# BurntSushi/aho-corasick

Hardware: NVIDIA H100
Metric: haystack_scan_throughput (higher is better)
Workload: dtype u8

## Files before the change

aho-corasick_b200/csrc/acb_api.cu:

```cuda
#include <cuda_runtime.h>

#include <algorithm>
#include <chrono>
#include <cstdio>
#include <cstdlib>
#include <cstring>
#include <atomic>
#include <pthread.h>
#include <condition_variable>
#include <functional>
#include <mutex>
#include <thread>
#include <new>
#include <optional>
#include <vector>

#include "../../include/acb200.h"
#include "../../include/acb200_debug.h"
#include "acb_build.hpp"
#include "acb_comm.hpp"
#include "acb_device.cuh"
#include "acb_plan.hpp"

using acb::DfaDev;
// ... 53 lines not shown
  cudaStream_t stream = nullptr, copy_stream = nullptr;
  cudaEvent_t ev0 = nullptr, ev1 = nullptr, ev2 = nullptr, ev3 = nullptr;
  DevBuf<uint64_t> d_keys[2];
  DevBuf<uint32_t> d_pids[2];
  uint64_t tuple_cap() const { return d_keys[0].cap; }
  DevBuf<unsigned long long> d_counter;
  PinnedBuf<unsigned long long> h_counter;
  DevBuf<uint8_t> d_temp;
  DevBuf<uint8_t> d_hay;
  DevBuf<uint64_t> d_scratch;
  DevBuf<uint8_t> d_flags;
  DevBuf<uint64_t> d_rec;
  PinnedBuf<uint64_t> h_rec;
  acg_stats stats{};
  PinnedBuf<uint8_t> h_stage[2];
  cudaEvent_t stage_ev[2] = {nullptr, nullptr};
  DevBuf<uint64_t> d_doc_offs;
  DevBuf<unsigned long long> d_doc_counts, d_doc_incl;
  DevBuf<uint8_t> d_doc_flags;
  DevBuf<uint64_t> d_rep;
  DevBuf<uint8_t> d_out;
  DevBuf<uint8_t> d_sdocs;
  DevBuf<uint64_t> d_soffs;
  DevBuf<uint64_t> d_held;
};

}

struct acg_dfa {
  HostDfa h;
  std::vector<uint16_t> depth16;
  acb::PrefilterPlan pf;
  uint32_t* d_bitmap = nullptr;
  uint2* d_amap = nullptr;
  bool has_empty = false;
  uint32_t max_list_len = 0;
  bool on_device = false;
  bool dev_touched = false;
  int device = -1;
  uint32_t* d_trans = nullptr;
  uint8_t* d_classes = nullptr;
  uint32_t* d_moff = nullptr;
  uint32_t* d_mpids = nullptr;
  uint32_t* d_plens = nullptr;
  uint16_t* d_depth16 = nullptr;
  DfaDev dev{};
  int engine_override = ACG_ENGINE_AUTO;
  uint64_t pipeline_chunk = 64ull << 20;
  mutable bool bytescan_inert = false;
  uint32_t experiment = 0;
  mutable std::mutex mu;
  static constexpr size_t kMaxWorkspaces = 4;
  mutable std::vector<Workspace*> ws_all, ws_free;
  mutable std::condition_variable ws_cv;
  mutable acg_stats last_stats{};
};

struct acg_streams {
  const acg_dfa* a = nullptr;
  uint64_t n = 0, back = 0;
  bool overlapping = false;
  bool replace = false;
  uint64_t* d_state = nullptr;
  uint8_t* d_tail = nullptr;
  uint64_t* d_rep = nullptr;
};
// ... 173 lines not shown
  std::vector<uint32_t>().swap(fp.edge_off);
  std::vector<uint8_t>().swap(fp.edge_class);
  std::vector<uint32_t>().swap(fp.edge_to);
  return ACG_OK;
}

int upload(acg_dfa* a) {
  int ndev = 0;
  if (cudaGetDeviceCount(&ndev) != cudaSuccess || ndev == 0) {
    cudaGetLastError();
    return ACG_E_NO_DEVICE;
  }
  CK(cudaGetDevice(&a->device));
  a->dev_touched = true;
  HostDfa& h = a->h;
  auto up = [&](auto** dptr, const void* src, size_t bytes) -> cudaError_t {
    cudaError_t e = cudaMalloc(reinterpret_cast<void**>(dptr), std::max<size_t>(bytes, 16));
    if (e != cudaSuccess) return e;
    if (bytes) e = cudaMemcpy(*dptr, src, bytes, cudaMemcpyHostToDevice);
    return e;
  };
  if (h.fill.valid) {
    int rc = fill_table_on_device(a);
    if (rc) return rc;
  } else {
    CK(up(&a->d_trans, h.trans.data(), h.trans.size() * 4));
  }
  CK(up(&a->d_classes, h.classes, 256));
  CK(up(&a->d_moff, h.match_offsets.data(), h.match_offsets.size() * 4));
  CK(up(&a->d_mpids, h.match_pids.data(), h.match_pids.size() * 4));
  CK(up(&a->d_plens, h.pattern_lens.data(), h.pattern_lens.size() * 4));
  CK(up(&a->d_depth16, a->depth16.data(), a->depth16.size() * 2));
  if (a->pf.supported && !a->pf.bitmap.empty()) CK(up(&a->d_bitmap, a->pf.bitmap.data(), a->pf.bitmap.size() * 4));
  if (a->pf.supported && !a->pf.amap.empty()) CK(up(&a->d_amap, a->pf.amap.data(), a->pf.amap.size() * 8));
  DfaDev& d = a->dev;
  d.trans = a->d_trans;
  d.classes = a->d_classes;
  d.match_offsets = a->d_moff;
  d.match_pids = a->d_mpids;
  d.pattern_lens = a->d_plens;
  d.depth16 = a->d_depth16;
  d.stride2 = h.stride2;
  d.max_match_id = h.max_match_id;
  d.start_unanchored_id = h.start_unanchored_id;
  d.start_anchored_id = h.start_anchored_id;
  d.max_pattern_len = uint32_t(std::min<uint64_t>(h.max_pattern_len, UINT32_MAX));
  d.min_pattern_len = uint32_t(std::min<uint64_t>(h.min_pattern_len, UINT32_MAX));
  d.amap = a->d_amap;
  acb::plan_device_fields(a->pf, d);
  a->on_device = true;
  return ACG_OK;
}

int reserve_tuples(Workspace& w, uint64_t cap) {
  return reserve_all(cap, w.d_keys[0], w.d_pids[0], w.d_keys[1], w.d_pids[1]);
}

template <class F>
int cub_call(Workspace& w, F f) {
  size_t tb = 0;
  CK(f(nullptr, tb));
  int rc = w.d_temp.reserve(std::max<size_t>(tb, 16));
  if (rc) return rc;
  tb = w.d_temp.cap;
  CK(f(w.d_temp, tb));
  return ACG_OK;
// ... 50 lines not shown
  if (const char* e = getenv("ACB_EMU_BUCKETSHIFT")) { shift = std::min<uint32_t>(uint32_t(atoi(e)), max_shift); min_shift = 1; }
  if (const char* e = getenv("ACB_EMU_BUCKETLOG")) log = std::min<uint32_t>(uint32_t(std::max(atoi(e), 0)), acb::kOrderLog);
#endif
  if (shift < min_shift) return b;
  while ((n_bytes >> shift) + 1 > acb::kMaxBuckets) {
    if (shift >= max_shift) return b;
    ++shift;
  }
  b.shift = shift;
  b.n = uint32_t((n_bytes >> shift) + 1);
  b.log = log;
  b.tie_bits = tie_bits;
  return b;
}

int enqueue_prefilter_range(const acg_dfa* a, const uint8_t* d_hay, uint64_t readable,
                            uint64_t span_start, uint64_t span_end, uint64_t scan_lo,
                            uint64_t scan_hi, int mode, int dev_sms, const BucketPlan& bp,
                            const DocBatch* docs) {
  Workspace& w = cur_ws();
  const acb::PrefilterPlan& pf = a->pf;
  const uintptr_t base = reinterpret_cast<uintptr_t>(d_hay);
  uint64_t lo = scan_lo + ((16 - ((base + scan_lo) & 15)) & 15);
  const uint64_t limit = std::min<uint64_t>(scan_hi, readable >= 20 ? readable - 20 : 0);
  uint64_t hi = lo;
  if (limit > lo) hi = lo + ((limit - lo) & ~15ull);
  if (lo > scan_hi) { lo = scan_hi; hi = scan_hi; }
  acb::PrefilterLaunch p;
  p.hay = d_hay;
  p.hay_len = readable;
  p.span_start = span_start;
  p.span_end = span_end;
  p.bitmap = a->d_bitmap;
  p.log_bits = pf.log_bits;
  p.k = pf.k;
  p.stride = pf.stride;
  p.geom = pf.wide ? 1 : 0;
  p.dyn = (a->experiment & ACG_EXP_STATIC_TILES) ? 0 : ((a->experiment & ACG_EXP_GLOBAL_TILES) ? 2 : 1);
  p.kmask = pf.kmask;
  p.fold = pf.fold;
  p.mult = pf.mult;
  p.mult3 = pf.mult3;
  p.key_shift = pf.key_shift;
  p.shift = pf.shift;
  p.dense = pf.dense ? 1 : 0;
  p.brute = pf.brute ? 1 : 0;
  p.mode = mode == 1 ? 1 : 0;
  p.first_only = mode == 2 ? 1 : 0;
  p.dup_shift = pf.dup_shift;
  p.scan_lo = scan_lo;
  p.scan_hi = scan_hi;
  p.region_lo = lo;
  p.region_hi = hi;
  p.keys = w.d_keys[0];
  p.pids = w.d_pids[0];
  p.counter = w.d_counter;
  p.cap = w.tuple_cap();
  p.bucket_shift = bp.shift;
  p.bucket_log = bp.log;
  p.bucket_slots = bp.slots();
  p.doc_offsets = docs ? docs->d_offsets : nullptr;
  p.n_docs = docs ? docs->n : 0;
  p.bs_n = 0;
  for (int i = 0; i < 3; ++i) { p.bs_needle[i] = 0; p.bs_back[i] = 0; }
  if (pf.bs_n && !a->bytescan_inert && !(a->experiment & ACG_EXP_NO_BYTESCAN)) {
    p.bs_n = pf.bs_n;
// ... 1745 lines not shown
    std::memcpy(h.classes, d->byte_classes, 256);
    h.max_special_id = d->max_special_id;
    h.max_match_id = d->max_match_id;
    h.start_unanchored_id = d->start_unanchored_id;
    h.start_anchored_id = d->start_anchored_id;
    const size_t nms = size_t(d->max_match_id >> d->stride2) - 1;
    h.match_offsets.assign(d->match_offsets, d->match_offsets + nms + 1);
    h.match_pids.assign(d->match_pids, d->match_pids + h.match_offsets[nms]);
    h.pattern_lens.assign(d->pattern_lens, d->pattern_lens + d->n_patterns);
    h.match_kind = int(d->match_kind);
    h.start_kind = int(d->start_kind);
    h.prefilter_kind = int(d->prefilter_kind);
    h.reported_kind = ACG_KIND_DFA;
    h.min_pattern_len = d->min_pattern_len;
    h.max_pattern_len = d->max_pattern_len;
    h.state_len = d->trans_len >> d->stride2;
    derive_metadata(a);
  } catch (const std::bad_alloc&) {
    delete a;
    return ACG_E_NOMEM;
  }
  int rc = upload(a);
  if (rc != ACG_OK && rc != ACG_E_NO_DEVICE) { acg_dfa_free(a); return rc; }
  *out = a;
  return ACG_OK;
}

void acg_dfa_free(acg_dfa* a) {
  if (!a) return;
  if (a->on_device || a->dev_touched) {
    DeviceGuard guard(a->device);
    for (Workspace* w : a->ws_all) { destroy_workspace(*w); delete w; }
    cudaFree(a->d_trans); cudaFree(a->d_classes); cudaFree(a->d_moff); cudaFree(a->d_mpids);
    cudaFree(a->d_plens); cudaFree(a->d_depth16); cudaFree(a->d_bitmap); cudaFree(a->d_amap);
  }
  delete a;
}

namespace {
int fetch_table(const acg_dfa* a) {
  HostDfa& h = const_cast<acg_dfa*>(a)->h;
  if (!h.fill.valid || !h.trans.empty()) return ACG_OK;
  if (!a->d_trans) return ACG_E_NO_DEVICE;
  std::lock_guard<std::mutex> lock(a->mu);
  if (!h.trans.empty()) return ACG_OK;
  DeviceGuard guard(a->device);
  std::vector<uint32_t> t(size_t(h.trans_len));
  if (cudaMemcpy(t.data(), a->d_trans, t.size() * 4, cudaMemcpyDeviceToHost) != cudaSuccess) {
    cudaGetLastError();
    return ACG_E_CUDA;
  }
  h.trans.swap(t);
  return ACG_OK;
}

}

int acg_dfa_table(const acg_dfa* a, acg_dfa_desc* o) {
  if (!a || !o) return ACG_E_INVALID_ARG;
  if (int rc = fetch_table(a)) return rc;
  const HostDfa& h = a->h;
  o->trans = h.trans.data();
  o->trans_len = h.trans.size();
  o->stride2 = h.stride2;
  o->alphabet_len = h.alphabet_len;
  std::memcpy(o->byte_classes, h.classes, 256);
  o->max_special_id = h.max_special_id;
// ... 14 lines not shown

uint64_t acg_dfa_state_len(const acg_dfa* a) { return a ? a->h.state_len : 0; }
int acg_kind(const acg_dfa* a) { return a ? a->h.reported_kind : 0; }
int acg_match_kind(const acg_dfa* a) { return a ? a->h.match_kind : 0; }
int acg_start_kind(const acg_dfa* a) { return a ? a->h.start_kind : 0; }
uint64_t acg_patterns_len(const acg_dfa* a) { return a ? a->h.pattern_lens.size() : 0; }
uint64_t acg_min_pattern_len(const acg_dfa* a) { return a ? a->h.min_pattern_len : 0; }
uint64_t acg_max_pattern_len(const acg_dfa* a) { return a ? a->h.max_pattern_len : 0; }
uint64_t acg_memory_usage(const acg_dfa* a) {
  if (!a) return 0;
  const HostDfa& h = a->h;
  return h.trans_len * 4 + (h.match_offsets.size() - 1) * 24 + h.match_pids.size() * 4 +
         h.pattern_lens.size() * 4;
}
int acg_prefilter_kind(const acg_dfa* a) { return a ? a->h.prefilter_kind : 0; }
int acg_packed_variant(const acg_dfa* a, int* fat, int* mask_len) {
  if (!a || !a->h.packed.active) return 0;
  if (fat) *fat = a->h.packed.fat;
  if (mask_len) *mask_len = a->h.packed.mask_len;
  return 1;
}

int acg_debug_prefilter_plan(const acg_dfa* a, acg_prefilter_plan* out) {
  if (!a || !out) return ACG_E_INVALID_ARG;
  const acb::PrefilterPlan& pf = a->pf;
  *out = acg_prefilter_plan{};
  out->supported = pf.supported ? 1 : 0;
  out->brute = pf.brute ? 1 : 0;
  out->dense = pf.dense ? 1 : 0;
  out->stride = int32_t(pf.stride);
  out->wide = pf.wide ? 1 : 0;
  out->k = pf.k; out->kmask = pf.kmask; out->fold = pf.fold;
  out->mult = pf.mult; out->mult3 = pf.mult3; out->key_shift = pf.key_shift; out->shift = pf.shift; out->log_bits = pf.log_bits;
  out->bitmap = pf.bitmap.data(); out->bitmap_words = pf.bitmap.size();
  out->amap = pf.amap.data(); out->amap_log = pf.amap_log;
  out->depth16 = a->depth16.data(); out->n_rows = a->depth16.size();
  out->dup_shift = pf.dup_shift;
  out->bs_n = (pf.bs_n && !a->bytescan_inert) ? pf.bs_n : 0;
  for (int i = 0; i < 3; ++i) { out->bs_byte[i] = pf.bs_byte[i]; out->bs_back[i] = pf.bs_back[i]; }
  return ACG_OK;
}

int acg_debug_set_pipeline_chunk(acg_dfa* a, uint64_t bytes) {
  if (!a || bytes < 4096 || (bytes & 4095)) return ACG_E_INVALID_ARG;
  a->pipeline_chunk = bytes;
  return ACG_OK;
}

int acg_debug_set_experiment(acg_dfa* a, uint32_t flags) {
  if (!a || (flags & ~uint32_t(ACG_EXP_KEY24 | ACG_EXP_STATIC_TILES | ACG_EXP_NO_BYTESCAN | ACG_EXP_GLOBAL_TILES))) return ACG_E_INVALID_ARG;
  std::lock_guard<std::mutex> lock(a->mu);
  const uint32_t changed = a->experiment ^ flags;
  a->experiment = flags;
  if (changed & ACG_EXP_KEY24) {
    const size_t old_words = a->pf.bitmap.size();
    a->pf = acb::plan_prefilter(a->h, a->depth16, (flags & ACG_EXP_KEY24) != 0);
    if (a->on_device && a->d_bitmap && a->pf.supported) {
      if (a->pf.bitmap.size() != old_words) return ACG_E_INVALID_ARG;
      DeviceGuard guard(a->device);
      if (cudaMemcpy(a->d_bitmap, a->pf.bitmap.data(), old_words * 4, cudaMemcpyHostToDevice) != cudaSuccess) {
        cudaGetLastError();
        return ACG_E_CUDA;
      }
    }
  }
  return ACG_OK;
}

int acg_set_engine(acg_dfa* a, int engine) {
  if (!a || engine < ACG_ENGINE_AUTO || engine > ACG_ENGINE_SEQUENTIAL) return ACG_E_INVALID_ARG;
  a->engine_override = engine;
  return ACG_OK;
}
static acg_stats stats_for(const acg_dfa* a) {
  if (tls_stats_owner == a) return tls_stats;
  std::lock_guard<std::mutex> lk(a->mu);
  return a->last_stats;
}
int acg_last_engine(const acg_dfa* a) { return a ? stats_for(a).engine : 0; }
int acg_last_stats(const acg_dfa* a, acg_stats* out) {
  if (!a || !out) return ACG_E_INVALID_ARG;
  *out = stats_for(a);
  return ACG_OK;
}

int acg_find_overlapping(const acg_dfa* a, const uint8_t* hay, uint64_t hay_len, uint64_t span_start,
                         uint64_t span_end, int anchored, acg_match* out, uint64_t cap,
                         uint64_t* n_out) {
  return overlapping_impl(a, hay, false, hay_len, span_start, span_end, anchored, out, cap, n_out,
                          nullptr, nullptr);
}
int acg_find_overlapping_dev(const acg_dfa* a, const void* d_hay, uint64_t hay_len,
                             uint64_t span_start, uint64_t span_end, acg_match* out, uint64_t cap,
// ... 600 lines not shown
```

aho-corasick_b200/csrc/acb_device.cuh:

```cuda
#pragma once
#include <cuda_runtime.h>
#include <stdint.h>

namespace acb {

constexpr int kTieBits = 24;
constexpr uint64_t kTieMask = (1ull << kTieBits) - 1;
constexpr uint64_t kInvalidKey = ~0ull;

struct MatchSpan {
  uint64_t start, end;
};
__host__ __device__ __forceinline__ MatchSpan decode_key(uint64_t key, uint32_t pid, int key_mode, uint64_t span_start,
                                                         const uint32_t* pattern_lens) {
  const uint64_t at = span_start + (key >> kTieBits);
  if (key_mode == 1) return MatchSpan{at, at + (key & kTieMask)};
  return MatchSpan{at - pattern_lens[pid], at};
}

struct TupleList {
  const uint64_t* keys;
  const uint32_t* pids;
  const uint32_t* pattern_lens;
  uint64_t n;
// ... 192 lines not shown
cudaError_t launch_stream_flush(const StreamLaunch& p, const uint64_t* ids, uint64_t n_ids,
                                const uint64_t* out_offsets, uint8_t* out, cudaStream_t s);

struct LookLaunch {
  StreamLaunch st;
  const uint64_t* ids;
  uint64_t n_rows;
  const uint64_t* cand_offsets;
  const uint8_t* cand_classes;
  uint64_t n_cands;
  uint64_t* keys;
  uint32_t* rows;
  uint64_t* skeys;
  uint32_t* srows;
  unsigned long long* heads;
  uint64_t* row_u;
  uint8_t* out;
  int sm_count;
};
cudaError_t launch_look_state(const DfaDev& dfa, const LookLaunch& p, cudaStream_t s);
cudaError_t launch_look_heads(const LookLaunch& p, cudaStream_t s);
cudaError_t launch_look_compact(const LookLaunch& p, cudaStream_t s);
cudaError_t launch_look_mask(const DfaDev& dfa, const LookLaunch& p, cudaStream_t s);
cudaError_t launch_look_copy(const LookLaunch& p, cudaStream_t s);

cudaError_t launch_check_offsets(const uint64_t* offs, uint64_t n_docs, uint64_t hay_len,
                                 unsigned long long* result, cudaStream_t s);

struct PrefilterLaunch {
  const uint8_t* hay;
  uint64_t hay_len;
  uint64_t span_start, span_end;
  const uint32_t* bitmap;
  uint32_t log_bits;
  uint32_t k;
  uint32_t stride;
  uint16_t geom;
  uint32_t kmask;
  uint32_t fold;
  uint32_t mult;
  uint32_t mult3;
  uint32_t shift;
  int dense;
  int brute;
  int mode;
  int first_only;
  uint32_t dup_shift;
  uint64_t scan_lo, scan_hi;
  uint64_t region_lo, region_hi;
  uint64_t* keys;
  uint32_t* pids;
  unsigned long long* counter;
  uint64_t cap;
  uint32_t dyn;
  uint32_t bs_n;
  uint32_t bs_needle[3];
  uint32_t bs_back[3];
  uint32_t key_shift;
  uint32_t bucket_shift;
  uint32_t bucket_log;
  uint64_t bucket_slots;
  const uint64_t* doc_offsets;
  uint64_t n_docs;
};
cudaError_t launch_prefilter(const DfaDev& dfa, const PrefilterLaunch& p, int sm_count, cudaStream_t s);
cudaError_t launch_bytescan(const DfaDev& dfa, const PrefilterLaunch& p, int sm_count, cudaStream_t s);
// ... 50 lines not shown
```

aho-corasick_b200/csrc/acb_fingerprint.cuh:

```cuda
#pragma once
#include <stdint.h>

#ifdef __CUDACC__
#define ACB_FP_FN __host__ __device__ __forceinline__
#else
#define ACB_FP_FN inline
#endif

namespace acb {

constexpr uint32_t kNarrowLogBits = 20, kWideLogBits = 17;
ACB_FP_FN constexpr uint32_t bloom_shift(uint32_t log_bits) { return 35 - log_bits; }
constexpr uint64_t kDenseGrams = 8192;
constexpr uint32_t kMult = 0x9E3779B1u;

ACB_FP_FN uint32_t bloom_hash2(uint32_t x) {
  x ^= x >> 16;
  x *= 0x7feb352du;
  x ^= x >> 15;
  x *= 0x846ca68bu;
  x ^= x >> 16;
  return x;
}

ACB_FP_FN uint32_t bloom_hash3(uint32_t x) {
  x ^= x >> 15;
  x *= 0x2c1b3c6du;
  x ^= x >> 12;
  x *= 0x297a2d39u;
  x ^= x >> 15;
  return x;
}

ACB_FP_FN uint32_t bloom_bit(uint32_t h, uint32_t sel, uint32_t shift) { return (h >> shift) * 8 + (sel & 7); }
ACB_FP_FN uint32_t key_mult(uint32_t mult3, uint32_t key_shift) { return mult3 << key_shift; }

ACB_FP_FN uint32_t dense_word(uint32_t lo, uint32_t shift) { return lo >> (shift + 2); }
ACB_FP_FN uint32_t dense_bit_a(uint32_t hi) { return hi & 31; }
ACB_FP_FN uint32_t dense_bit_b(uint32_t hi) { return (hi >> 5) & 31; }

ACB_FP_FN int bit_width(uint64_t v) { int b = 0; for (; v; v >>= 1) ++b; return b; }

ACB_FP_FN uint32_t amap_log_for(uint64_t n_keys) { return uint32_t(bit_width((n_keys * 4 - 1) | 15)); }
ACB_FP_FN uint32_t amap_slot(uint32_t key, uint32_t amap_shift) { return bloom_hash3(key) >> amap_shift; }
ACB_FP_FN uint32_t amap_next(uint32_t slot, uint32_t amap_mask) { return (slot + 1) & amap_mask; }
// ... 4 lines not shown
```

aho-corasick_b200/csrc/acb_plan.hpp:

```cpp
#pragma once
#include <algorithm>

#include "acb_build.hpp"
#include "acb_device.cuh"
#include "acb_fingerprint.cuh"

namespace acb {

struct PrefilterPlan {
  bool supported = false;
  uint32_t k = 0, kmask = 0, fold = 0, mult = 1, mult3 = 1, shift = 0, log_bits = 0;
  uint32_t stride = 1;
  uint32_t key_shift = 8;
  bool wide = false;
  bool brute = false;
  uint32_t dup_shift = 0;
  std::vector<uint32_t> bitmap;
  bool dense = false;
  std::vector<uint64_t> amap;
  uint32_t amap_log = 0;
  uint32_t bs_n = 0;
  uint8_t bs_byte[3] = {0, 0, 0};
  uint8_t bs_back[3] = {0, 0, 0};
};

namespace plan_detail {

inline void set_bit(std::vector<uint32_t>& bm, uint32_t bit) { bm[bit >> 5] |= 1u << (bit & 31); }
inline uint32_t test_bit(const std::vector<uint32_t>& bm, uint32_t bit) { return (bm[bit >> 5] >> (bit & 31)) & 1u; }

inline std::vector<uint32_t> bloom_bitmap(const std::vector<uint32_t>& grams, uint32_t log_bits) {
  const uint32_t shift = bloom_shift(log_bits);
  std::vector<uint32_t> bm(size_t(1) << (log_bits - 5), 0u);
  for (uint32_t g : grams) {
    const uint32_t h1 = g * kMult, h2 = bloom_hash2(g);
    set_bit(bm, bloom_bit(h1, h1, shift));
    set_bit(bm, bloom_bit(h2, h2, shift));
  }
  return bm;
}

struct DenseBits { uint32_t word, mask; };
inline DenseBits dense_bits(uint32_t g, uint32_t shift) {
  const uint64_t prod = uint64_t(g) * kMult;
  const uint32_t hi = uint32_t(prod >> 32);
  return {dense_word(uint32_t(prod), shift), (1u << dense_bit_a(hi)) | (1u << dense_bit_b(hi))};
}

struct Alphabets {
  std::vector<uint8_t> at[4];
// ... 110 lines not shown
    std::fill(pf.bitmap.begin(), pf.bitmap.end(), 0u);
    for (uint32_t g : best_set) { const DenseBits d = dense_bits(g, pf.shift); pf.bitmap[d.word] |= d.mask; }
    const Alphabets alpha = alphabets(best_set, pf.k);
    fill = double(count_passes([&](auto& next) {
             uint32_t g = 0;
             for (uint32_t j = 0; j < pf.k; ++j) g |= uint32_t(alpha.at[j][(next() >> 33) % alpha.at[j].size()]) << (8 * j);
             const DenseBits d = dense_bits(g, pf.shift);
             return uint32_t((pf.bitmap[d.word] & d.mask) == d.mask);
           })) / kTrials;
  }
  pf.brute = fill > 0.25;
  pf.supported = true;
  if (!pf.brute && pf.k == 4 && !dense) {
    std::vector<uint32_t> g3;
    g3.reserve(best_set.size() * 2);
    const uint32_t f3 = pf.fold & 0x00FFFFFFu;
    for (uint32_t g : best_set) {
      g3.push_back((g & 0x00FFFFFFu) | f3);
      g3.push_back((g >> 8) | f3);
    }
    std::sort(g3.begin(), g3.end());
    g3.erase(std::unique(g3.begin(), g3.end()), g3.end());
    const Alphabets alpha = alphabets(g3, 3);
    const double n_bits_set = double(g3.size()) + 2.0 * double(best_set.size());
    const double true3 = double(g3.size()) / alpha.space;
    const double pass1 = n_bits_set / double(uint64_t(1) << pf.log_bits) + true3;
    if (pass1 < 0.07) {
      pf.stride = 2;
      pf.wide = n_bits_set / double(uint64_t(1) << kWideLogBits) + true3 < 0.01;
      if (pf.wide) {
        pf.log_bits = kWideLogBits;
        pf.shift = bloom_shift(kWideLogBits);
        pf.bitmap = bloom_bitmap(best_set, kWideLogBits);
      }
      pf.key_shift = key24 ? 8 : 5;
      std::vector<uint32_t> keys1;
      if (key24) {
        keys1 = g3;
      } else {
        for (const Item& it : level[4]) {
          const uint32_t g = it.gram;
          keys1.push_back(((g & 0x00FFFFFFu) | f3) | (((g >> 24) & 7u) << 24));
          uint32_t xs = 0;
          if (it.row >= 2 && (it.row << s2) <= h.max_match_id) {
            const uint32_t lo = h.match_offsets[it.row - 2], hi = h.match_offsets[it.row - 1];
            if (lo < hi && h.pattern_lens[h.match_pids[lo]] == 4) xs = 0xFF;
          }
          if (xs != 0xFF)
            for_each_edge(it.row, [&](uint32_t b, uint32_t nr) {
              if (depth16[nr] == 5) xs |= 1u << (b & 7);
            });
          for (uint32_t x = 0; x < 8; ++x)
            if (xs >> x & 1) keys1.push_back(((g >> 8) | f3) | (x << 24));
        }
        std::sort(keys1.begin(), keys1.end());
        keys1.erase(std::unique(keys1.begin(), keys1.end()), keys1.end());
      }
      static const uint32_t kCand[] = {0x1B873593u, 0x27D4EB2Fu, 0x165667B1u, 0x9E3779B1u, 0x2C1B3C6Du,
                                       0xB5297A4Du, 0x85EBCA6Bu, 0x5BD1E995u, 0x7FEB352Du, 0xCC9E2D51u,
                                       0x1B56C4E9u, 0xC2B2AE35u};
      auto key_bit = [&](uint32_t g, uint32_t m) { return bloom_bit(g * key_mult(m, pf.key_shift), g, pf.shift); };
      uint32_t best_m = kCand[0];
      uint64_t best_pass = UINT64_MAX;
      std::vector<uint32_t> trial;
      for (uint32_t m : kCand) {
        trial = pf.bitmap;
        for (uint32_t g : keys1) set_bit(trial, key_bit(g, m));
        const uint64_t pass = count_passes([&](auto& next) {
          const uint64_t x = next();
          const uint32_t r = uint32_t(x >> 33);
          uint32_t g = uint32_t(alpha.at[0][r % alpha.at[0].size()]) |
                       uint32_t(alpha.at[1][(r >> 10) % alpha.at[1].size()]) << 8 |
                       uint32_t(alpha.at[2][(r >> 20) % alpha.at[2].size()]) << 16;
          if (!key24) g |= uint32_t((x >> 20) & 7) << 24;
          return test_bit(trial, key_bit(g, m));
        });
        if (pass < best_pass) { best_pass = pass; best_m = m; }
      }
      pf.mult3 = best_m;
      for (uint32_t g : keys1) set_bit(pf.bitmap, key_bit(g, best_m));
    }
  }
  pf.dense = !pf.brute && dense;
  const std::vector<Item>& paths = level[pf.k];
  if (!paths.empty() && paths.size() <= (4u << 20)) {
    pf.amap_log = amap_log_for(paths.size());
    pf.amap.assign(size_t(1) << pf.amap_log, 0ull);
    const uint32_t shift = 32 - pf.amap_log, mask = (1u << pf.amap_log) - 1;
    for (const Item& it : paths) {
      const uint32_t key = it.gram & pf.kmask;
      uint32_t slot = amap_slot(key, shift);
      while (pf.amap[slot] != 0 && uint32_t(pf.amap[slot]) != key) slot = amap_next(slot, mask);
      pf.amap[slot] = amap_entry(key, it.row << s2);
    }
  }
  if (h.prefilter_kind == kPreStartBytes || h.prefilter_kind == kPreRareBytes) {
    if (h.pre_n) {
      if (std::all_of(h.pre_back, h.pre_back + h.pre_n, [](uint8_t back) { return back == 0; })) {
        pf.bs_n = h.pre_n;
        std::copy(h.pre_byte, h.pre_byte + h.pre_n, pf.bs_byte);
      }
    } else if (h.prefilter_kind == kPreStartBytes && !level[1].empty() && grams[1].size() <= 3) {
      pf.bs_n = uint32_t(grams[1].size());
      std::copy(grams[1].begin(), grams[1].end(), pf.bs_byte);
    }
  }
  return pf;
}

inline void plan_device_fields(const PrefilterPlan& pf, DfaDev& d) {
  d.amap_shift = pf.amap_log ? 32 - pf.amap_log : 0;
  d.amap_mask = pf.amap_log ? (1u << pf.amap_log) - 1 : 0;
  d.amap_k = pf.k;
// ... 5 lines not shown
```

aho-corasick_b200/csrc/acb_prefilter.cu:

```cuda
#include "acb_device.cuh"
#include "acb_fingerprint.cuh"
#ifndef ACB_PTX_HEADER
#define ACB_PTX_HEADER "acb_ptx.cuh"
#endif
#include ACB_PTX_HEADER

#include <cstdio>
#include <cstdlib>
#include <type_traits>

#include <cub/device/device_scan.cuh>
#include <cub/device/device_select.cuh>

namespace acb {
namespace {

enum : int { kGeomNarrow = 0, kGeomWide = 1 };
template <int GEOM> struct PfGeom {
  static constexpr int kThreads = GEOM == kGeomNarrow ? 1024 : 512;
  static constexpr int kWarps = kThreads / 32;
  static constexpr int kGroups = GEOM == kGeomNarrow ? 2 : 4;
  static constexpr int kTile = kGroups * 512;
  static constexpr int kStageBytes = kTile + 16;
  static constexpr int kMinCtas = GEOM == kGeomWide ? 2 : 1;
  static constexpr uint32_t kLogBits = GEOM == kGeomWide ? kWideLogBits : kNarrowLogBits;
};
template <bool DENSE> struct PfCfg {
  static constexpr int kSlots = 256;
  static constexpr int kQ2 = DENSE ? 64 : 96;
};

#ifdef ACB_EMULATE
static const uint32_t kWinShift = getenv("ACB_EMU_WINSHIFT") ? (uint32_t)atoi(getenv("ACB_EMU_WINSHIFT")) : 31u;
#else
constexpr uint32_t kWinShift = 31;
#endif

constexpr int kPfStages = 2;

template <int GEOM, int STRIDE> struct PfPass {
  static constexpr bool kPair = STRIDE == 2 && GEOM == kGeomNarrow;
  static constexpr int kStages = kPair ? 1 : kPfStages;
  static constexpr int kGroups = PfGeom<GEOM>::kGroups * (kPair ? 2 : 1);
  static constexpr int kTile = kGroups * 512;
  static_assert(kStages * (kTile + 16) <= kPfStages * PfGeom<GEOM>::kStageBytes, "a step's tiles fit the warp's ring");
};

template <bool BUCKETED = true>
struct Emitter {
  uint64_t* g_keys;
  uint32_t* g_pids;
  unsigned long long* g_counter;
  uint64_t cap;
  uint32_t bucket_shift, bucket_log;
  uint64_t bucket_slots;
  __device__ __forceinline__ void emit(uint64_t key, uint32_t pid) {
    const unsigned m = __activemask();
    const int leader = __ffs(m) - 1;
    const int lane = threadIdx.x & 31;
    const bool bucketed = BUCKETED && bucket_shift != 0;
    unsigned long long* cnt = g_counter;
// ... 97 lines not shown
}

template <int MODE, class EM>
__device__ __forceinline__ void verify_at(const DfaDev& d, const PrefilterLaunch& p, const uint8_t* s_cls,
                                          uint64_t s, EM& em) {
  if (d.amap != nullptr) {
    const uint32_t sid = anchor_lookup(d, p, s);
    if (sid != 0) verify_from<MODE>(d, p, s_cls, s, sid, d.amap_k, em);
  } else {
    verify_from<MODE>(d, p, s_cls, s, d.start_unanchored_id, 0, em);
  }
}

template <uint32_t SHIFT>
__device__ __forceinline__ bool bloom_test(const uint32_t* s_bitmap, uint32_t h) {
  const uint32_t byte = reinterpret_cast<const uint8_t*>(s_bitmap)[h >> SHIFT];
  const uint32_t rep = byte * 0x01010101u;
  return (__funnelshift_r(rep, rep, h) & 1u) != 0;
}

template <int MODE, bool MASKED, bool DENSE, int STRIDE, int GEOM, int DYN = 0>
__global__ void __launch_bounds__(PfGeom<GEOM>::kThreads, PfGeom<GEOM>::kMinCtas)
prefilter_kernel(DfaDev d, PrefilterLaunch p) {
  static_assert(STRIDE == 1 || STRIDE == 2, "fingerprint stride");
  static_assert(GEOM == kGeomNarrow || STRIDE == 2, "the 2 KiB tile needs the stride-2 first stage (32 hit bits per lane)");
  constexpr bool ANCH = DENSE;
  constexpr int kPfThreads = PfGeom<GEOM>::kThreads;
  constexpr int kPfWarps = PfGeom<GEOM>::kWarps;
  constexpr int kRingBytes = kPfStages * PfGeom<GEOM>::kStageBytes;
  constexpr int kStages = PfPass<GEOM, STRIDE>::kStages;
  constexpr int kPfTile = PfPass<GEOM, STRIDE>::kTile;
  constexpr int kPfStageBytes = kPfTile + 16;
  constexpr int kGroups = PfPass<GEOM, STRIDE>::kGroups;
  constexpr int kPfSlots = PfCfg<DENSE>::kSlots;
  constexpr int kPfQ2 = PfCfg<ANCH>::kQ2;
  constexpr uint32_t kBloomShift = bloom_shift(PfGeom<GEOM>::kLogBits);
  using Q2Entry = typename std::conditional<ANCH, uint2, uint32_t>::type;
  ACB_DYNAMIC_SMEM(smem_raw);
  unsigned char* s_ring = smem_raw;
  uint64_t* s_bars = reinterpret_cast<uint64_t*>(s_ring + kPfWarps * kRingBytes);
  uint32_t* s_tile_of = reinterpret_cast<uint32_t*>(s_bars + kPfWarps * kPfStages);
  uint32_t* s_next_tile = s_tile_of + kPfWarps * kPfStages;
  Q2Entry* s_queue2 = reinterpret_cast<Q2Entry*>(s_next_tile + 4);
  uint16_t* s_slots = reinterpret_cast<uint16_t*>(s_queue2 + kPfWarps * kPfQ2);
  uint32_t* s_bitmap = reinterpret_cast<uint32_t*>(s_slots + kPfWarps * kPfSlots);
  __shared__ uint8_t s_cls[256];

  const int tid = threadIdx.x;
  const int lane = tid & 31;
  const int warp = tid >> 5;
  const uint32_t bitmap_words = p.brute ? 0u : (1u << (p.log_bits - 5));
  for (uint32_t i = tid; i < bitmap_words; i += kPfThreads) s_bitmap[i] = p.bitmap[i];
  if (tid < 256) s_cls[tid] = d.classes[tid];
  if (tid < kPfWarps * kPfStages) ptx::mbar_init(ptx::smem_addr(&s_bars[tid]), 1);
  if (tid == 0) {
    *reinterpret_cast<uint64_t*>(s_next_tile) = DYN == 2 ? (uint64_t)blockIdx.x << 32 : 0ull;
    s_next_tile[2] = 0xFFFFFFFEu;
  }
  ptx::mbar_init_fence();
  ptx::fence_proxy_async();
  __syncthreads();

  Emitter<DYN != 2> em{p.keys, p.pids, p.counter, p.cap, p.bucket_shift, p.bucket_log, p.bucket_slots};
  unsigned long long cand_total = 0;

  if (blockIdx.x == 0) {
    const uint64_t tail_lo = (p.region_hi > p.region_lo && !p.brute) ? p.region_hi - (STRIDE - 1) : p.region_hi;
    const uint64_t head_n = p.region_lo - p.scan_lo;
    const uint64_t tail_n = p.scan_hi > tail_lo ? p.scan_hi - tail_lo : 0;
    for (uint64_t i = tid; i < head_n + tail_n; i += kPfThreads) {
      const uint64_t s = i < head_n ? p.scan_lo + i : tail_lo + (i - head_n);
      verify_at<MODE>(d, p, s_cls, s, em);
    }
  }

  const uint64_t n_blocks16 = (p.region_hi - p.region_lo) >> 4;
  const uint64_t per_cta = (n_blocks16 + gridDim.x - 1) / gridDim.x;
  const uint64_t b0 = (uint64_t)blockIdx.x * per_cta;
  const uint64_t b1 = min(b0 + per_cta, n_blocks16);
  const uint64_t split_lo = p.region_lo + (b0 << 4);
  const uint64_t split_hi = b0 < b1 ? p.region_lo + (b1 << 4) : split_lo;

  if (p.brute) {
    for (uint64_t s = split_lo + tid; s < split_hi; s += kPfThreads) verify_at<MODE>(d, p, s_cls, s, em);
    if (tid == 0 && split_hi > split_lo) atomicAdd(p.counter + 1, (unsigned long long)(split_hi - split_lo));
// ... 274 lines not shown
            for (int u = 0; u < 2; ++u) {
              if (look[u]) {
                while (ent[u].y != 0 && ent[u].x != key2[u]) {
                  slot2[u] = amap_next(slot2[u], d.amap_mask);
                  ent[u] = __ldg(d.amap + slot2[u]);
                }
                sid2[u] = ent[u].y;
                pass2[u] = sid2[u] != 0;
              }
              const uint32_t bal = __ballot_sync(0xffffffffu, pass2[u]);
              if (bal) {
                if (pass2[u]) q2[q2len + __popc(bal & lt)] = make_uint2(rel2[u], sid2[u]);
                q2len += __popc(bal);
                if (q2len > (uint32_t)(kPfQ2 - 32)) drain2();
              }
            }
          }
        } else
        for (uint32_t base = 0; base < n_items; base += 32) {
          const uint32_t w = base + lane;
          const uint32_t j = STRIDE == 2 ? (w & 1u) : 0u;
          bool pass = false;
          uint32_t e = 0;
          if (w < n_items) {
            const uint32_t raw = slots[STRIDE == 2 ? (w >> 1) : w];
            e = hit_offset(raw & 31u, raw >> 5);
            if (STRIDE == 2 && e < j) {
              pass = !region_first;
            } else {
              const uint32_t off = e - j;
              const uint32_t sa = tile_a + (off & ~3u);
              uint32_t gram = __funnelshift_r(ptx::lds32(sa), ptx::lds32(sa + 4), (off & 3) * 8);
              if (MASKED) gram = (gram | fold) & kmask;
              if (STRIDE == 2) pass = bloom_test<kBloomShift>(s_bitmap, gram * mult) && bloom_test<kBloomShift>(s_bitmap, bloom_hash2(gram));
              else pass = bloom_test<kBloomShift>(s_bitmap, bloom_hash2(gram));
            }
          }
          const uint32_t bal = __ballot_sync(0xffffffffu, pass);
          if (bal) {
            if (pass) {
              const uint32_t rel = wrel + e - j;
              if constexpr (!ANCH) q2[q2len + __popc(bal & lt)] = rel;
            }
            q2len += __popc(bal);
            if (q2len > (uint32_t)(kPfQ2 - 32)) drain2();
          }
        }
      }
    }
    __syncwarp();
    if (lane == 0) {
      if constexpr (DYN) draw(stage);
      else if (t + kStages * kPfWarps < n_tiles) issue(t + kStages * kPfWarps, stage, t + (kStages + 1) * kPfWarps);
    }
    if constexpr (DYN && kStages == 1) __syncwarp();
  }
  if constexpr (DYN == 2) { if (lane == 0) publish(); }
  if (q2len) drain2();
  if (lane == 0 && cand_total) atomicAdd(p.counter + 1, cand_total);
}

constexpr int kBsThreads = 512;
constexpr int kBsWarps = kBsThreads / 32;
constexpr int kBsQueue = 128;

template <int MODE>
__global__ void __launch_bounds__(kBsThreads, 2) bytescan_kernel(DfaDev d, PrefilterLaunch p) {
// ... 300 lines not shown
  __shared__ unsigned long long s_part[kCompactThreads];
  const uint32_t b = blockIdx.x;
  const int tid = threadIdx.x;
  unsigned long long part = 0;
  for (uint32_t i = tid; i < b && i < o.n_buckets; i += kCompactThreads) part += min(o.bucket_count[i], (unsigned long long)o.bucket_cap);
  s_part[tid] = part;
  __syncthreads();
  uint64_t dst = 0;
  for (int i = 0; i < kCompactThreads; ++i) dst += s_part[i];
  const uint64_t n = b < o.n_buckets ? min(o.bucket_count[b], (unsigned long long)o.bucket_cap) : *o.overflow_count;
  const uint64_t src = b < o.n_buckets ? (uint64_t)b * o.bucket_cap : o.bucket_slots;
  for (uint64_t j = tid; j < n; j += kCompactThreads) {
    o.keys_out[dst + j] = o.keys_in[src + j];
    o.pids_out[dst + j] = o.pids_in[src + j];
  }
}

}

cudaError_t launch_prefilter(const DfaDev& dfa, const PrefilterLaunch& p, int sm_count, cudaStream_t s) {
  const bool dense = p.dense != 0;
  const int geom = p.stride == 2 ? p.geom : kGeomNarrow;
  if (geom < kGeomNarrow || geom > kGeomWide) return cudaErrorInvalidValue;
  const uint32_t want_log = geom == kGeomWide ? PfGeom<kGeomWide>::kLogBits : PfGeom<kGeomNarrow>::kLogBits;
  if (!p.brute && (p.log_bits != want_log || p.shift != bloom_shift(want_log))) return cudaErrorInvalidValue;
  const size_t bitmap_bytes = p.brute ? 0 : (size_t(1) << (p.log_bits - 3));
  static const int kThreadsOf[2] = {PfGeom<0>::kThreads, PfGeom<1>::kThreads};
  static const int kStageOf[2] = {PfGeom<0>::kStageBytes, PfGeom<1>::kStageBytes};
  const int threads = kThreadsOf[geom];
  const int warps = threads / 32;
  const int stage_bytes = kStageOf[geom];
  const int tile = geom == kGeomWide ? PfPass<kGeomWide, 2>::kTile
                   : p.stride == 2 ? PfPass<kGeomNarrow, 2>::kTile : PfPass<kGeomNarrow, 1>::kTile;
  const int q2_bytes = dense ? PfCfg<true>::kQ2 * 8 : PfCfg<false>::kQ2 * 4;
  const int slot_bytes = PfCfg<false>::kSlots * 2;
  const size_t smem = size_t(warps) * (kPfStages * stage_bytes + kPfStages * 12 + q2_bytes + slot_bytes) + 16 + bitmap_bytes;
  if (smem > 227 * 1024 - 1024) return cudaErrorInvalidValue;
  const bool masked = p.fold != 0 || p.kmask != 0xFFFFFFFFu;
  using KernT = void (*)(DfaDev, PrefilterLaunch);
#define ACB_PF_ROW(M, K, D)                                                                                 \
  {prefilter_kernel<M, K, false, 1, kGeomNarrow, D>, prefilter_kernel<M, K, true, 1, kGeomNarrow, D>, \
   prefilter_kernel<M, K, false, 2, kGeomNarrow, D>, prefilter_kernel<M, K, false, 2, kGeomWide, D>}
  static const KernT table[2][2][3][4] = {
      {{ACB_PF_ROW(0, false, 0), ACB_PF_ROW(0, false, 1), ACB_PF_ROW(0, false, 2)},
       {ACB_PF_ROW(0, true, 0), ACB_PF_ROW(0, true, 1), ACB_PF_ROW(0, true, 2)}},
      {{ACB_PF_ROW(1, false, 0), ACB_PF_ROW(1, false, 1), ACB_PF_ROW(1, false, 2)},
       {ACB_PF_ROW(1, true, 0), ACB_PF_ROW(1, true, 1), ACB_PF_ROW(1, true, 2)}}};
#undef ACB_PF_ROW
  if (p.dyn > 2) return cudaErrorInvalidValue;
  if (p.stride == 2 && dense) return cudaErrorInvalidValue;
  int variant = dense ? 1 : 0;
  if (p.stride == 2) variant = geom == kGeomWide ? 3 : 2;
  KernT kern = table[p.mode ? 1 : 0][masked ? 1 : 0][p.dyn][variant];
#ifdef ACB_EMULATE
  if (getenv("ACB_EMU_TRACE")) fprintf(stderr, "launch_prefilter variant %d dyn %d threads %d smem %zu\n", variant, (int)p.dyn, threads, smem);
#endif
  cudaError_t e = cudaFuncSetAttribute(kern, cudaFuncAttributeMaxDynamicSharedMemorySize, (int)smem);
  if (e != cudaSuccess) return e;
  int per_sm = 1;
  e = cudaOccupancyMaxActiveBlocksPerMultiprocessor(&per_sm, kern, threads, smem);
  if (e != cudaSuccess) return e;
  if (per_sm < 1) per_sm = 1;
  uint64_t grid = (uint64_t)sm_count * per_sm;
  const uint64_t cta_step = uint64_t(warps) * tile;
  const uint64_t warp_steps = ((p.region_hi - p.region_lo) + cta_step - 1) / cta_step;
  if (grid > warp_steps) grid = warp_steps ? warp_steps : 1;
  ACB_LAUNCH(kern, (unsigned)grid, threads, smem, s, dfa, p);
  return cudaGetLastError();
}
// ... 59 lines not shown
```

include/acb200_debug.h:

```cpp
#ifndef ACB200_DEBUG_H
#define ACB200_DEBUG_H

#include "acb200.h"

#ifdef __cplusplus
extern "C" {
#endif

typedef struct {
  int32_t supported;
  int32_t brute;
  int32_t dense;
  int32_t stride;
  int32_t wide;
  uint32_t k;
  uint32_t kmask, fold, mult, mult3, shift, log_bits;
  const uint32_t* bitmap;
  uint64_t bitmap_words;
  const uint64_t* amap;
  uint32_t amap_log;
  const uint16_t* depth16;
  uint64_t n_rows;
  uint32_t dup_shift;
  uint32_t key_shift;
  uint32_t bs_n;
  uint8_t bs_byte[3];
  uint8_t bs_back[3];
} acg_prefilter_plan;

int acg_debug_prefilter_plan(const acg_dfa* dfa, acg_prefilter_plan* out);

int acg_debug_set_pipeline_chunk(acg_dfa* dfa, uint64_t bytes);

#define ACG_EXP_KEY24 8u
#define ACG_EXP_STATIC_TILES 32u
#define ACG_EXP_GLOBAL_TILES 16u
#define ACG_EXP_NO_BYTESCAN 64u
int acg_debug_set_experiment(acg_dfa* dfa, uint32_t flags);

#ifdef __cplusplus
}
#endif
#endif
```

Measured before the change: 2136.

## Split narrow stride-2 prefilter into separate stage-1 and stage-2 bloom bitmaps

For the narrow geometry with stride 2, the single shared bloom bitmap is split into two: the stage-1 key bitmap keeps only the key bits, and a separate 2^17-bit bitmap holds the two-hash gram bloom used for the second-stage test. Separating them is meant to lower the false-positive rate of each stage, since the two sets no longer share one bitmap. The cost is extra shared memory for the second bitmap, offset by shrinking per-warp slot buffers from 256 to 64 entries. This may affect occupancy and slot overflow behaviour.

```diff
diff --git a/aho-corasick_b200/csrc/acb_api.cu b/aho-corasick_b200/csrc/acb_api.cu
--- a/aho-corasick_b200/csrc/acb_api.cu
+++ b/aho-corasick_b200/csrc/acb_api.cu
@@ -109,6 +109,7 @@
   std::vector<uint16_t> depth16;
   acb::PrefilterPlan pf;
   uint32_t* d_bitmap = nullptr;
+  uint32_t* d_bitmap2 = nullptr;
   uint2* d_amap = nullptr;
   bool has_empty = false;
   uint32_t max_list_len = 0;
@@ -348,6 +349,7 @@
   CK(up(&a->d_plens, h.pattern_lens.data(), h.pattern_lens.size() * 4));
   CK(up(&a->d_depth16, a->depth16.data(), a->depth16.size() * 2));
   if (a->pf.supported && !a->pf.bitmap.empty()) CK(up(&a->d_bitmap, a->pf.bitmap.data(), a->pf.bitmap.size() * 4));
+  if (a->pf.supported && !a->pf.bitmap2.empty()) CK(up(&a->d_bitmap2, a->pf.bitmap2.data(), a->pf.bitmap2.size() * 4));
   if (a->pf.supported && !a->pf.amap.empty()) CK(up(&a->d_amap, a->pf.amap.data(), a->pf.amap.size() * 8));
   DfaDev& d = a->dev;
   d.trans = a->d_trans;
@@ -464,6 +466,7 @@
   p.span_start = span_start;
   p.span_end = span_end;
   p.bitmap = a->d_bitmap;
+  p.bitmap2 = a->d_bitmap2;
   p.log_bits = pf.log_bits;
   p.k = pf.k;
   p.stride = pf.stride;
@@ -2275,7 +2278,7 @@
     DeviceGuard guard(a->device);
     for (Workspace* w : a->ws_all) { destroy_workspace(*w); delete w; }
     cudaFree(a->d_trans); cudaFree(a->d_classes); cudaFree(a->d_moff); cudaFree(a->d_mpids);
-    cudaFree(a->d_plens); cudaFree(a->d_depth16); cudaFree(a->d_bitmap); cudaFree(a->d_amap);
+    cudaFree(a->d_plens); cudaFree(a->d_depth16); cudaFree(a->d_bitmap); cudaFree(a->d_bitmap2); cudaFree(a->d_amap);
   }
   delete a;
 }
@@ -2356,12 +2359,24 @@
   out->wide = pf.wide ? 1 : 0;
   out->k = pf.k; out->kmask = pf.kmask; out->fold = pf.fold;
   out->mult = pf.mult; out->mult3 = pf.mult3; out->key_shift = pf.key_shift; out->shift = pf.shift; out->log_bits = pf.log_bits;
-  out->bitmap = pf.bitmap.data(); out->bitmap_words = pf.bitmap.size();
+  const std::vector<uint32_t>& bm = pf.both.empty() ? pf.bitmap : pf.both;
+  out->bitmap = bm.data(); out->bitmap_words = bm.size();
   out->amap = pf.amap.data(); out->amap_log = pf.amap_log;
   out->depth16 = a->depth16.data(); out->n_rows = a->depth16.size();
   out->dup_shift = pf.dup_shift;
   out->bs_n = (pf.bs_n && !a->bytescan_inert) ? pf.bs_n : 0;
   for (int i = 0; i < 3; ++i) { out->bs_byte[i] = pf.bs_byte[i]; out->bs_back[i] = pf.bs_back[i]; }
+  return ACG_OK;
+}
+
+int acg_debug_prefilter_stages(const acg_dfa* a, acg_prefilter_stages* out) {
+  if (!a || !out) return ACG_E_INVALID_ARG;
+  const acb::PrefilterPlan& pf = a->pf;
+  *out = acg_prefilter_stages{};
+  out->stage1 = pf.bitmap.data(); out->stage1_words = pf.bitmap.size();
+  if (!pf.bitmap2.empty()) {
+    out->stage2 = pf.bitmap2.data(); out->stage2_words = pf.bitmap2.size(); out->stage2_log_bits = acb::kStage2LogBits;
+  }
   return ACG_OK;
 }
 
@@ -2377,12 +2392,13 @@
   const uint32_t changed = a->experiment ^ flags;
   a->experiment = flags;
   if (changed & ACG_EXP_KEY24) {
-    const size_t old_words = a->pf.bitmap.size();
+    const size_t old_words = a->pf.bitmap.size(), old_words2 = a->pf.bitmap2.size();
     a->pf = acb::plan_prefilter(a->h, a->depth16, (flags & ACG_EXP_KEY24) != 0);
     if (a->on_device && a->d_bitmap && a->pf.supported) {
-      if (a->pf.bitmap.size() != old_words) return ACG_E_INVALID_ARG;
+      if (a->pf.bitmap.size() != old_words || a->pf.bitmap2.size() != old_words2) return ACG_E_INVALID_ARG;
       DeviceGuard guard(a->device);
-      if (cudaMemcpy(a->d_bitmap, a->pf.bitmap.data(), old_words * 4, cudaMemcpyHostToDevice) != cudaSuccess) {
+      if (cudaMemcpy(a->d_bitmap, a->pf.bitmap.data(), old_words * 4, cudaMemcpyHostToDevice) != cudaSuccess ||
+          (old_words2 && cudaMemcpy(a->d_bitmap2, a->pf.bitmap2.data(), old_words2 * 4, cudaMemcpyHostToDevice) != cudaSuccess)) {
         cudaGetLastError();
         return ACG_E_CUDA;
       }
diff --git a/aho-corasick_b200/csrc/acb_device.cuh b/aho-corasick_b200/csrc/acb_device.cuh
--- a/aho-corasick_b200/csrc/acb_device.cuh
+++ b/aho-corasick_b200/csrc/acb_device.cuh
@@ -248,6 +248,7 @@
   uint64_t hay_len;
   uint64_t span_start, span_end;
   const uint32_t* bitmap;
+  const uint32_t* bitmap2;
   uint32_t log_bits;
   uint32_t k;
   uint32_t stride;
diff --git a/aho-corasick_b200/csrc/acb_fingerprint.cuh b/aho-corasick_b200/csrc/acb_fingerprint.cuh
--- a/aho-corasick_b200/csrc/acb_fingerprint.cuh
+++ b/aho-corasick_b200/csrc/acb_fingerprint.cuh
@@ -11,6 +11,8 @@
 
 constexpr uint32_t kNarrowLogBits = 20, kWideLogBits = 17;
 ACB_FP_FN constexpr uint32_t bloom_shift(uint32_t log_bits) { return 35 - log_bits; }
+constexpr uint32_t kStage2LogBits = 17;
+constexpr uint32_t kStage2Shift = bloom_shift(kStage2LogBits);
 constexpr uint64_t kDenseGrams = 8192;
 constexpr uint32_t kMult = 0x9E3779B1u;
 
diff --git a/aho-corasick_b200/csrc/acb_plan.hpp b/aho-corasick_b200/csrc/acb_plan.hpp
--- a/aho-corasick_b200/csrc/acb_plan.hpp
+++ b/aho-corasick_b200/csrc/acb_plan.hpp
@@ -16,6 +16,8 @@
   bool brute = false;
   uint32_t dup_shift = 0;
   std::vector<uint32_t> bitmap;
+  std::vector<uint32_t> bitmap2;
+  std::vector<uint32_t> both;
   bool dense = false;
   std::vector<uint64_t> amap;
   uint32_t amap_log = 0;
@@ -192,6 +194,9 @@
         pf.log_bits = kWideLogBits;
         pf.shift = bloom_shift(kWideLogBits);
         pf.bitmap = bloom_bitmap(best_set, kWideLogBits);
+      } else {
+        pf.bitmap.assign(size_t(1) << (pf.log_bits - 5), 0u);
+        pf.bitmap2 = bloom_bitmap(best_set, kStage2LogBits);
       }
       pf.key_shift = key24 ? 8 : 5;
       std::vector<uint32_t> keys1;
@@ -239,6 +244,10 @@
       }
       pf.mult3 = best_m;
       for (uint32_t g : keys1) set_bit(pf.bitmap, key_bit(g, best_m));
+      if (!pf.wide) {
+        pf.both = bloom_bitmap(best_set, pf.log_bits);
+        for (size_t i = 0; i < pf.both.size(); ++i) pf.both[i] |= pf.bitmap[i];
+      }
     }
   }
   pf.dense = !pf.brute && dense;
diff --git a/aho-corasick_b200/csrc/acb_prefilter.cu b/aho-corasick_b200/csrc/acb_prefilter.cu
--- a/aho-corasick_b200/csrc/acb_prefilter.cu
+++ b/aho-corasick_b200/csrc/acb_prefilter.cu
@@ -25,8 +25,9 @@
   static constexpr int kMinCtas = GEOM == kGeomWide ? 2 : 1;
   static constexpr uint32_t kLogBits = GEOM == kGeomWide ? kWideLogBits : kNarrowLogBits;
 };
-template <bool DENSE> struct PfCfg {
-  static constexpr int kSlots = 256;
+__host__ __device__ constexpr bool own_stage2_filter(int geom, int stride) { return stride == 2 && geom == kGeomNarrow; }
+template <bool DENSE, bool OWN2 = false> struct PfCfg {
+  static constexpr int kSlots = OWN2 ? 64 : 256;
   static constexpr int kQ2 = DENSE ? 64 : 96;
 };
 
@@ -190,7 +191,8 @@
   constexpr int kPfTile = PfPass<GEOM, STRIDE>::kTile;
   constexpr int kPfStageBytes = kPfTile + 16;
   constexpr int kGroups = PfPass<GEOM, STRIDE>::kGroups;
-  constexpr int kPfSlots = PfCfg<DENSE>::kSlots;
+  constexpr bool kOwn2 = own_stage2_filter(GEOM, STRIDE);
+  constexpr int kPfSlots = PfCfg<DENSE, kOwn2>::kSlots;
   constexpr int kPfQ2 = PfCfg<ANCH>::kQ2;
   constexpr uint32_t kBloomShift = bloom_shift(PfGeom<GEOM>::kLogBits);
   using Q2Entry = typename std::conditional<ANCH, uint2, uint32_t>::type;
@@ -202,6 +204,8 @@
   Q2Entry* s_queue2 = reinterpret_cast<Q2Entry*>(s_next_tile + 4);
   uint16_t* s_slots = reinterpret_cast<uint16_t*>(s_queue2 + kPfWarps * kPfQ2);
   uint32_t* s_bitmap = reinterpret_cast<uint32_t*>(s_slots + kPfWarps * kPfSlots);
+  uint32_t* s_stage2 = kOwn2 ? s_bitmap + (1u << (PfGeom<GEOM>::kLogBits - 5)) : s_bitmap;
+  constexpr uint32_t kStage2BloomShift = kOwn2 ? kStage2Shift : kBloomShift;
   __shared__ uint8_t s_cls[256];
 
   const int tid = threadIdx.x;
@@ -209,6 +213,8 @@
   const int warp = tid >> 5;
   const uint32_t bitmap_words = p.brute ? 0u : (1u << (p.log_bits - 5));
   for (uint32_t i = tid; i < bitmap_words; i += kPfThreads) s_bitmap[i] = p.bitmap[i];
+  if (kOwn2 && !p.brute)
+    for (uint32_t i = tid; i < (1u << (kStage2LogBits - 5)); i += kPfThreads) s_stage2[i] = p.bitmap2[i];
   if (tid < 256) s_cls[tid] = d.classes[tid];
   if (tid < kPfWarps * kPfStages) ptx::mbar_init(ptx::smem_addr(&s_bars[tid]), 1);
   if (tid == 0) {
@@ -549,7 +555,7 @@
               const uint32_t sa = tile_a + (off & ~3u);
               uint32_t gram = __funnelshift_r(ptx::lds32(sa), ptx::lds32(sa + 4), (off & 3) * 8);
               if (MASKED) gram = (gram | fold) & kmask;
-              if (STRIDE == 2) pass = bloom_test<kBloomShift>(s_bitmap, gram * mult) && bloom_test<kBloomShift>(s_bitmap, bloom_hash2(gram));
+              if (STRIDE == 2) pass = bloom_test<kStage2BloomShift>(s_stage2, gram * mult) && bloom_test<kStage2BloomShift>(s_stage2, bloom_hash2(gram));
               else pass = bloom_test<kBloomShift>(s_bitmap, bloom_hash2(gram));
             }
           }
@@ -916,9 +922,13 @@
   const int stage_bytes = kStageOf[geom];
   const int tile = geom == kGeomWide ? PfPass<kGeomWide, 2>::kTile
                    : p.stride == 2 ? PfPass<kGeomNarrow, 2>::kTile : PfPass<kGeomNarrow, 1>::kTile;
+  const bool own2 = own_stage2_filter(geom, (int)p.stride) && !p.brute;
+  if (own2 && p.bitmap2 == nullptr) return cudaErrorInvalidValue;
   const int q2_bytes = dense ? PfCfg<true>::kQ2 * 8 : PfCfg<false>::kQ2 * 4;
-  const int slot_bytes = PfCfg<false>::kSlots * 2;
-  const size_t smem = size_t(warps) * (kPfStages * stage_bytes + kPfStages * 12 + q2_bytes + slot_bytes) + 16 + bitmap_bytes;
+  const int slot_bytes = (own2 ? PfCfg<false, true>::kSlots : PfCfg<false>::kSlots) * 2;
+  const size_t bitmap2_bytes = own2 ? (size_t(1) << (kStage2LogBits - 3)) : 0;
+  const size_t smem = size_t(warps) * (kPfStages * stage_bytes + kPfStages * 12 + q2_bytes + slot_bytes) + 16 +
+                      bitmap_bytes + bitmap2_bytes;
   if (smem > 227 * 1024 - 1024) return cudaErrorInvalidValue;
   const bool masked = p.fold != 0 || p.kmask != 0xFFFFFFFFu;
   using KernT = void (*)(DfaDev, PrefilterLaunch);
diff --git a/include/acb200_debug.h b/include/acb200_debug.h
--- a/include/acb200_debug.h
+++ b/include/acb200_debug.h
@@ -30,6 +30,15 @@
 
 int acg_debug_prefilter_plan(const acg_dfa* dfa, acg_prefilter_plan* out);
 
+typedef struct {
+  const uint32_t* stage1;
+  uint64_t stage1_words;
+  const uint32_t* stage2;
+  uint64_t stage2_words;
+  uint32_t stage2_log_bits;
+} acg_prefilter_stages;
+int acg_debug_prefilter_stages(const acg_dfa* dfa, acg_prefilter_stages* out);
+
 int acg_debug_set_pipeline_chunk(acg_dfa* dfa, uint64_t bytes);
 
 #define ACG_EXP_KEY24 8u
```

After: 2141, median of 6. About the same (+0.2%).
